# facebookresearch/actionmesh

Measured on NVIDIA H100. Metric: denoiser_steps_per_sec, higher is better.
Workload: dtype bf16

## Files before the change

### actionmesh_b200/csrc/attention.cu

```cuda
#include "common.cuh"
#include "ptx.cuh"
#include "attention.cuh"

namespace amb {

constexpr int ATT_BQ = 128;
constexpr int ATT_BK = 128;
constexpr int ATT_THREADS = 384;
constexpr int ATT_STAGES = 2;

template <int D>
struct AttnSmem {
  static constexpr int BOX_BYTES = 128 * 128;
  static constexpr int Q_BYTES = (D / 64) * BOX_BYTES;
  static constexpr int KV_BYTES = (D / 64) * BOX_BYTES;
  static constexpr int Q_OFF = 0;
  static constexpr int K_OFF = Q_BYTES;
  static constexpr int V_OFF = K_OFF + ATT_STAGES * KV_BYTES;
  static constexpr int BAR_OFF = V_OFF + ATT_STAGES * KV_BYTES;
  static constexpr int NUM_BARS = 1 + 4 * ATT_STAGES;
  static constexpr int TOTAL = BAR_OFF + NUM_BARS * 8 + 1024;
};

template <int D>
__device__ __forceinline__ void qk_issue(float* sc, uint32_t sq_addr, uint32_t sk_addr) {
#pragma unroll
  for (int k = 0; k < D / 16; ++k) {
    const uint32_t off = (k >> 2) * AttnSmem<D>::BOX_BYTES + (k & 3) * 32;
    wgmma_ss_n128(sc, make_desc_kmajor_sw128(sq_addr + off), make_desc_kmajor_sw128(sk_addr + off), k > 0 ? 1u : 0u);
  }
  wgmma_commit();
}

template <int D>
__device__ __forceinline__ void pv_issue(float* o, const uint32_t* pk, uint32_t sv_addr) {
#pragma unroll
  for (int kk = 0; kk < ATT_BK / 16; ++kk) {
    const uint64_t vdesc = make_desc_mnmajor_sw128(sv_addr + kk * 2048, AttnSmem<D>::BOX_BYTES);
    if constexpr (D == 128) wgmma_rs_n128_tb(o, pk + 4 * kk, vdesc, 1u);
    else wgmma_rs_n64_tb(o, pk + 4 * kk, vdesc, 1u);
  }
  wgmma_commit();
}

__device__ __forceinline__ void softmax_tile(float* sc, int valid, int q, float c, float& m_a, float& m_b, float& l_a,
                                             float& l_b, float& al_a, float& al_b) {
  if (valid < ATT_BK) {
#pragma unroll
    for (int i = 0; i < 16; ++i) {
      const int key = 8 * i + 2 * q;
      if (key >= valid) sc[4 * i] = sc[4 * i + 2] = -INFINITY;
      if (key + 1 >= valid) sc[4 * i + 1] = sc[4 * i + 3] = -INFINITY;
    }
  }
  float mx_a = m_a, mx_b = m_b;
#pragma unroll
  for (int i = 0; i < 16; ++i) {
    mx_a = fmaxf(mx_a, fmaxf(sc[4 * i], sc[4 * i + 1]));
    mx_b = fmaxf(mx_b, fmaxf(sc[4 * i + 2], sc[4 * i + 3]));
  }
  mx_a = fmaxf(mx_a, __shfl_xor_sync(0xffffffffu, mx_a, 1));
  mx_b = fmaxf(mx_b, __shfl_xor_sync(0xffffffffu, mx_b, 1));
  mx_a = fmaxf(mx_a, __shfl_xor_sync(0xffffffffu, mx_a, 2));
  mx_b = fmaxf(mx_b, __shfl_xor_sync(0xffffffffu, mx_b, 2));
  al_a = ex2_approx((m_a - mx_a) * c);
  al_b = ex2_approx((m_b - mx_b) * c);
  m_a = mx_a;
  m_b = mx_b;
  const float mb_a = m_a * c, mb_b = m_b * c;
  float ts_a = 0.f, ts_b = 0.f;
#pragma unroll
  for (int i = 0; i < 16; ++i) {
    sc[4 * i] = ex2_approx(fmaf(sc[4 * i], c, -mb_a));
    sc[4 * i + 1] = ex2_approx(fmaf(sc[4 * i + 1], c, -mb_a));
    sc[4 * i + 2] = ex2_approx(fmaf(sc[4 * i + 2], c, -mb_b));
    sc[4 * i + 3] = ex2_approx(fmaf(sc[4 * i + 3], c, -mb_b));
    ts_a += sc[4 * i] + sc[4 * i + 1];
    ts_b += sc[4 * i + 2] + sc[4 * i + 3];
  }
  l_a = l_a * al_a + ts_a;
  l_b = l_b * al_b + ts_b;
}

__device__ __forceinline__ void pack_p(uint32_t* pk, const float* sc) {
#pragma unroll
  for (int i = 0; i < 16; ++i) {
    pk[2 * i] = pack_bf16(sc[4 * i], sc[4 * i + 1]);
    pk[2 * i + 1] = pack_bf16(sc[4 * i + 2], sc[4 * i + 3]);
  }
}

template <int D>
__global__ void __launch_bounds__(ATT_THREADS, 1)
flash_attn_fwd_kernel(const __grid_constant__ CUtensorMap tmQ, const __grid_constant__ CUtensorMap tmK,
                      const __grid_constant__ CUtensorMap tmV, const AttnParams p) {
  using L = AttnSmem<D>;
  constexpr int DH = D / 64;
  extern __shared__ uint8_t smem_raw[];
  uint8_t* smem = reinterpret_cast<uint8_t*>((reinterpret_cast<uintptr_t>(smem_raw) + 1023) & ~uintptr_t(1023));
  uint64_t* q_full = reinterpret_cast<uint64_t*>(smem + L::BAR_OFF);
  uint64_t* k_full = q_full + 1;
  uint64_t* v_full = k_full + ATT_STAGES;
  uint64_t* k_empty = v_full + ATT_STAGES;
  uint64_t* v_empty = k_empty + ATT_STAGES;

  const int wg = __shfl_sync(0xffffffffu, threadIdx.x >> 7, 0);
  const int warp = threadIdx.x >> 5;
  const int lane = threadIdx.x & 31;
  const int q0 = blockIdx.x * ATT_BQ;
  const int head = blockIdx.y;
  const int batch = blockIdx.z;
  const int tiles_per_chunk = (p.sk_chunk + ATT_BK - 1) / ATT_BK;
  const int n_kv = p.kv_chunks * tiles_per_chunk;

  if (threadIdx.x == 0) {
    tma_prefetch_desc(&tmQ);
    tma_prefetch_desc(&tmK);
    tma_prefetch_desc(&tmV);
    mbar_init(q_full, 1);
    for (int s = 0; s < ATT_STAGES; ++s) {
      mbar_init(&k_full[s], 1);
      mbar_init(&v_full[s], 1);
      mbar_init(&k_empty[s], 8);
      mbar_init(&v_empty[s], 8);
    }
    fence_mbar_init();
  }
  __syncthreads();

  if (wg == 0) {
    reg_dealloc<24>();
    if (warp == 0) {
      if (elect_one()) {
        mbar_expect_tx(q_full, L::Q_BYTES);
        for (int c = 0; c < DH; ++c)
          tma_load_4d(smem + L::Q_OFF + c * L::BOX_BYTES, &tmQ, q_full, c * 64, q0, head, batch, kEvictFirst);
      }
      __syncwarp();
      int s = 0;
      uint32_t phase = 0;
      for (int j = 0; j < n_kv; ++j) {
        const int chunk = j / tiles_per_chunk;
        const int key0 = (j - chunk * tiles_per_chunk) * ATT_BK;
        mbar_wait(&k_empty[s], phase ^ 1);
        if (elect_one()) {
          uint8_t* sk = smem + L::K_OFF + s * L::KV_BYTES;
          mbar_expect_tx(&k_full[s], L::KV_BYTES);
          for (int c = 0; c < DH; ++c)
            tma_load_5d(sk + c * L::BOX_BYTES, &tmK, &k_full[s], c * 64, key0, head, batch, chunk, kEvictLast);
        }
        __syncwarp();
        mbar_wait(&v_empty[s], phase ^ 1);
        if (elect_one()) {
          uint8_t* sv = smem + L::V_OFF + s * L::KV_BYTES;
          mbar_expect_tx(&v_full[s], L::KV_BYTES);
          for (int c = 0; c < DH; ++c)
            tma_load_5d(sv + c * L::BOX_BYTES, &tmV, &v_full[s], c * 64, key0, head, batch, chunk, kEvictLast);
        }
        __syncwarp();
        if (++s == ATT_STAGES) { s = 0; phase ^= 1; }
      }
      for (int j = 0; j < ATT_STAGES; ++j) {
        mbar_wait(&k_empty[s], phase ^ 1);
        mbar_wait(&v_empty[s], phase ^ 1);
        if (++s == ATT_STAGES) { s = 0; phase ^= 1; }
      }
    }
  } else {
    reg_alloc<240>();
    const int q = lane & 3;
    const int r_local = (wg - 1) * 64 + (warp & 3) * 16 + (lane >> 2);
    const uint32_t sq_addr = smem_u32(smem + L::Q_OFF) + (wg - 1) * 64 * 128;
    const uint32_t sk_addr = smem_u32(smem + L::K_OFF);
    const uint32_t sv_addr = smem_u32(smem + L::V_OFF);
    const float c = p.scale_log2;
    const int last_valid = p.sk_chunk - (tiles_per_chunk - 1) * ATT_BK;
    const uint32_t my_turn = wg, other_turn = 3 - wg;

    float o[D / 2];
#pragma unroll
    for (int i = 0; i < D / 2; ++i) o[i] = 0.f;
    float m_a = -INFINITY, m_b = -INFINITY;
    float l_a = 0.f, l_b = 0.f;
    float al_a, al_b;
    float sc[64];
    uint32_t pk[32];

    mbar_wait_watched(q_full, 0);
    mbar_wait_watched(&k_full[0], 0);
    if (wg == 2) named_bar_sync(my_turn, 256);
    wgmma_fence();
    qk_issue<D>(sc, sq_addr, sk_addr);
    named_bar_arrive(other_turn, 256);
    wgmma_wait<0>();
#pragma unroll
    for (int i = 0; i < 64; ++i) reg_fence(sc[i]);
    __syncwarp();
    if (lane == 0) mbar_arrive(&k_empty[0]);
    int jn = tiles_per_chunk == 1 ? 0 : 1;
    softmax_tile(sc, tiles_per_chunk == 1 ? last_valid : ATT_BK, q, c, m_a, m_b, l_a, l_b, al_a, al_b);
    pack_p(pk, sc);

    int s = 0;
    uint32_t phase = 0;
    for (int j = 0; j + 1 < n_kv; ++j) {
      int sn = s + 1;
      uint32_t phn = phase;
      if (sn == ATT_STAGES) { sn = 0; phn ^= 1; }
      mbar_wait_watched(&k_full[sn], phn);
      mbar_wait_watched(&v_full[s], phase);
      named_bar_sync(my_turn, 256);
      wgmma_fence();
      qk_issue<D>(sc, sq_addr, sk_addr + sn * L::KV_BYTES);
      pv_issue<D>(o, pk, sv_addr + s * L::KV_BYTES);
      named_bar_arrive(other_turn, 256);
      wgmma_wait<1>();
#pragma unroll
      for (int i = 0; i < 64; ++i) reg_fence(sc[i]);
      __syncwarp();
      if (lane == 0) mbar_arrive(&k_empty[sn]);
      softmax_tile(sc, jn == tiles_per_chunk - 1 ? last_valid : ATT_BK, q, c, m_a, m_b, l_a, l_b, al_a, al_b);
      if (++jn == tiles_per_chunk) jn = 0;
      wgmma_wait<0>();
#pragma unroll
      for (int i = 0; i < D / 2; ++i) reg_fence(o[i]);
      __syncwarp();
      if (lane == 0) mbar_arrive(&v_empty[s]);
#pragma unroll
      for (int i = 0; i < D / 8; ++i) {
        o[4 * i] *= al_a;
        o[4 * i + 1] *= al_a;
        o[4 * i + 2] *= al_b;
        o[4 * i + 3] *= al_b;
      }
      pack_p(pk, sc);
      s = sn;
      phase = phn;
    }

    mbar_wait_watched(&v_full[s], phase);
    named_bar_sync(my_turn, 256);
    wgmma_fence();
    pv_issue<D>(o, pk, sv_addr + s * L::KV_BYTES);
    if (wg == 1) named_bar_arrive(other_turn, 256);
    wgmma_wait<0>();
#pragma unroll
    for (int i = 0; i < D / 2; ++i) reg_fence(o[i]);
    __syncwarp();
    if (lane == 0) mbar_arrive(&v_empty[s]);

    l_a += __shfl_xor_sync(0xffffffffu, l_a, 1);
    l_b += __shfl_xor_sync(0xffffffffu, l_b, 1);
    l_a += __shfl_xor_sync(0xffffffffu, l_a, 2);
    l_b += __shfl_xor_sync(0xffffffffu, l_b, 2);
    const float inv_a = 1.0f / l_a, inv_b = 1.0f / l_b;
    const int qr_a = q0 + r_local, qr_b = qr_a + 8;
    __nv_bfloat16* obase = p.o + (long long)batch * p.o_stride_b + (long long)head * p.o_stride_h + 2 * q;
#pragma unroll
    for (int i = 0; i < D / 8; ++i) {
      if (qr_a < p.sq)
        *reinterpret_cast<uint32_t*>(obase + (long long)qr_a * p.o_stride_s + 8 * i) = pack_bf16(o[4 * i] * inv_a, o[4 * i + 1] * inv_a);
      if (qr_b < p.sq)
        *reinterpret_cast<uint32_t*>(obase + (long long)qr_b * p.o_stride_s + 8 * i) = pack_bf16(o[4 * i + 2] * inv_b, o[4 * i + 3] * inv_b);
    }
  }
}

template <int D>
static int launch_attn(const amb_attn_args* a, cudaStream_t stream) {
  using L = AttnSmem<D>;
  CUtensorMap tmQ, tmK, tmV;
  int r = encode_attn_maps(a, D, ATT_BQ, ATT_BK, ATT_BK, &tmQ, &tmK, &tmV);
  if (r) return r;
  const AttnParams p = make_attn_params(a);
  dim3 grid((a->sq + ATT_BQ - 1) / ATT_BQ, a->heads, a->batch);
  auto kern = flash_attn_fwd_kernel<D>;
  r = ensure_smem_optin(kern, L::TOTAL);
  if (r) return r;
  kern<<<grid, ATT_THREADS, L::TOTAL, stream>>>(tmQ, tmK, tmV, p);
  AMB_CHECK_CUDA(cudaGetLastError());
  return AMB_OK;
}

}

using namespace amb;

extern "C" int amb_flash_attn_fwd(const amb_attn_args* a, amb_stream_t stream) {
  AMB_CHECK_ARG(a && a->q && a->k && a->v && a->o, "flash_attn: null pointer");
  AMB_CHECK_ARG(a->batch > 0 && a->heads > 0 && a->sq > 0 && a->sk > 0, "flash_attn: bad shape b=%d h=%d sq=%d sk=%d",
                a->batch, a->heads, a->sq, a->sk);
  AMB_CHECK_ARG(a->head_dim == 128 || a->head_dim == 64, "flash_attn: head_dim %d unsupported (64 or 128)", a->head_dim);
  AMB_CHECK_ARG(a->q_stride_s % 8 == 0 && a->k_stride_s % 8 == 0 && a->v_stride_s % 8 == 0 && a->o_stride_s % 8 == 0 &&
                    a->q_stride_h % 8 == 0 && a->k_stride_h % 8 == 0 && a->v_stride_h % 8 == 0 && a->o_stride_h % 8 == 0 &&
                    a->q_stride_b % 8 == 0 && a->k_stride_b % 8 == 0 && a->v_stride_b % 8 == 0 && a->o_stride_b % 8 == 0,
                "flash_attn: strides must be multiples of 8 elements (16 bytes)");
  AMB_CHECK_ARG(a->kv_chunks <= 1 || (a->sk_chunk > 0 && (int64_t)a->sk_chunk * a->kv_chunks == a->sk),
                "flash_attn: kv_chunks * sk_chunk must equal sk");
  AMB_CHECK_ARG(a->batch <= 65535 && a->heads <= 65535, "flash_attn: grid limits");
  cudaStream_t s = (cudaStream_t)stream;
  if (a->head_dim == 64) return launch_attn<64>(a, s);
  return launch_attn<128>(a, s);
}
```

### actionmesh_b200/csrc/ptx.cuh

```cuda
#pragma once
#include <cstdint>
#include <cuda_runtime.h>
#include <cuda_bf16.h>

namespace amb {

__device__ __forceinline__ uint32_t smem_u32(const void* p) {
  return static_cast<uint32_t>(__cvta_generic_to_shared(p));
}
__device__ __forceinline__ uint32_t lane_id() { return threadIdx.x & 31; }

__device__ __forceinline__ bool elect_one() {
  uint32_t pred = 0;
  asm volatile(
      "{\n\t.reg .pred P;\n\t"
      "elect.sync _|P, 0xffffffff;\n\t"
      "selp.u32 %0, 1, 0, P;\n\t}\n"
      : "=r"(pred));
  return pred != 0;
}

__device__ __forceinline__ void mbar_init(uint64_t* bar, uint32_t count) {
  asm volatile("mbarrier.init.shared::cta.b64 [%0], %1;" ::"r"(smem_u32(bar)), "r"(count) : "memory");
}
__device__ __forceinline__ void fence_mbar_init() {
  asm volatile("fence.mbarrier_init.release.cluster;" ::: "memory");
}
__device__ __forceinline__ void fence_proxy_async_smem() {
  asm volatile("fence.proxy.async.shared::cta;" ::: "memory");
}
__device__ __forceinline__ void mbar_expect_tx(uint64_t* bar, uint32_t bytes) {
  asm volatile("mbarrier.arrive.expect_tx.shared::cta.b64 _, [%0], %1;" ::"r"(smem_u32(bar)), "r"(bytes)
               : "memory");
}
__device__ __forceinline__ void mbar_arrive(uint64_t* bar) {
  asm volatile("mbarrier.arrive.shared::cta.b64 _, [%0];" ::"r"(smem_u32(bar)) : "memory");
}
__device__ __forceinline__ uint32_t mbar_try_wait(uint64_t* bar, uint32_t parity) {
  uint32_t ok;
  asm volatile(
      "{\n\t.reg .pred P;\n\t"
      "mbarrier.try_wait.parity.shared::cta.b64 P, [%1], %2;\n\t"
      "selp.u32 %0, 1, 0, P;\n\t}\n"
      : "=r"(ok)
      : "r"(smem_u32(bar)), "r"(parity)
      : "memory");
  return ok;
}
__device__ __forceinline__ void mbar_arrive_cluster(uint64_t* bar, uint32_t cta) {
  asm volatile(
      "{\n\t.reg .b32 ra;\n\t"
      "mapa.shared::cluster.u32 ra, %0, %1;\n\t"
      "mbarrier.arrive.shared::cluster.b64 _, [ra];\n\t}\n"
      ::"r"(smem_u32(bar)), "r"(cta)
      : "memory");
}

__device__ __forceinline__ uint32_t cluster_ctarank() {
  uint32_t r;
  asm volatile("mov.u32 %0, %%cluster_ctarank;" : "=r"(r));
  return r;
}
__device__ __forceinline__ void cluster_sync() {
  asm volatile("barrier.cluster.arrive.release;\n\tbarrier.cluster.wait.acquire;" ::: "memory");
}
__device__ __forceinline__ uint64_t globaltimer_ns() {
  uint64_t t;
  asm volatile("mov.u64 %0, %%globaltimer;" : "=l"(t));
  return t;
}
#ifndef AMB_WAIT_TIMEOUT_NS
#define AMB_WAIT_TIMEOUT_NS 4000000000ull
#endif
#ifndef AMB_WAIT_TIMEOUT_PRINT
#define AMB_WAIT_TIMEOUT_PRINT 0
#endif
__device__ __forceinline__ void mbar_wait(uint64_t* bar, uint32_t parity) {
  if (mbar_try_wait(bar, parity)) return;
  uint64_t t0 = globaltimer_ns();
  uint32_t spins = 0;
  while (!mbar_try_wait(bar, parity)) {
    if ((++spins & 0xfff) == 0 && globaltimer_ns() - t0 > AMB_WAIT_TIMEOUT_NS) {
#if AMB_WAIT_TIMEOUT_PRINT
      printf("amb: mbarrier wait timeout block=(%d,%d,%d) thread=%d bar=%u parity=%u\n", blockIdx.x, blockIdx.y,
             blockIdx.z, threadIdx.x, smem_u32(bar), parity);
#endif
      __trap();
    }
  }
}
__device__ __forceinline__ void mbar_wait_watched(uint64_t* bar, uint32_t parity) {
  while (!mbar_try_wait(bar, parity)) {
  }
}

__device__ __forceinline__ void tma_prefetch_desc(const void* tmap) {
  asm volatile("prefetch.tensormap [%0];" ::"l"(reinterpret_cast<uint64_t>(tmap)) : "memory");
}
constexpr uint64_t kEvictNormal = 0x1000000000000000ull;
constexpr uint64_t kEvictFirst = 0x12F0000000000000ull;
constexpr uint64_t kEvictLast = 0x14F0000000000000ull;

__device__ __forceinline__ void tma_load_2d(void* dst, const void* tmap, uint64_t* bar, int c0, int c1,
                                            uint64_t hint) {
  asm volatile(
      "cp.async.bulk.tensor.2d.shared::cluster.global.mbarrier::complete_tx::bytes.L2::cache_hint"
      " [%0], [%1, {%3, %4}], [%2], %5;"
      :
      : "r"(smem_u32(dst)), "l"(reinterpret_cast<uint64_t>(tmap)), "r"(smem_u32(bar)), "r"(c0), "r"(c1), "l"(hint)
      : "memory");
}
__device__ __forceinline__ void tma_load_2d_multicast(void* dst, const void* tmap, uint64_t* bar, int c0, int c1,
                                                      uint16_t cta_mask, uint64_t hint) {
  asm volatile(
      "cp.async.bulk.tensor.2d.shared::cluster.global.mbarrier::complete_tx::bytes.multicast::cluster.L2::cache_hint"
      " [%0], [%1, {%4, %5}], [%2], %3, %6;"
      :
      : "r"(smem_u32(dst)), "l"(reinterpret_cast<uint64_t>(tmap)), "r"(smem_u32(bar)), "h"(cta_mask), "r"(c0), "r"(c1),
        "l"(hint)
      : "memory");
}
__device__ __forceinline__ void tma_load_4d(void* dst, const void* tmap, uint64_t* bar, int c0, int c1, int c2,
                                            int c3, uint64_t hint) {
  asm volatile(
      "cp.async.bulk.tensor.4d.shared::cluster.global.mbarrier::complete_tx::bytes.L2::cache_hint"
      " [%0], [%1, {%3, %4, %5, %6}], [%2], %7;"
      :
      : "r"(smem_u32(dst)), "l"(reinterpret_cast<uint64_t>(tmap)), "r"(smem_u32(bar)), "r"(c0), "r"(c1), "r"(c2),
        "r"(c3), "l"(hint)
      : "memory");
}

__device__ __forceinline__ void tma_load_5d(void* dst, const void* tmap, uint64_t* bar, int c0, int c1, int c2,
                                            int c3, int c4, uint64_t hint) {
  asm volatile(
      "cp.async.bulk.tensor.5d.shared::cluster.global.mbarrier::complete_tx::bytes.L2::cache_hint"
      " [%0], [%1, {%3, %4, %5, %6, %7}], [%2], %8;"
      :
      : "r"(smem_u32(dst)), "l"(reinterpret_cast<uint64_t>(tmap)), "r"(smem_u32(bar)), "r"(c0), "r"(c1), "r"(c2),
        "r"(c3), "r"(c4), "l"(hint)
      : "memory");
}

__device__ __forceinline__ void wgmma_fence() { asm volatile("wgmma.fence.sync.aligned;" ::: "memory"); }
__device__ __forceinline__ void wgmma_commit() { asm volatile("wgmma.commit_group.sync.aligned;" ::: "memory"); }
template <int N>
__device__ __forceinline__ void wgmma_wait() {
  asm volatile("wgmma.wait_group.sync.aligned %0;" ::"n"(N) : "memory");
}
__device__ __forceinline__ void reg_fence(float& r) { asm volatile("" : "+f"(r)::"memory"); }

__device__ __forceinline__ uint64_t make_smem_desc(uint32_t saddr, uint32_t lbo_bytes, uint32_t sbo_bytes) {
  uint64_t d = 0;
  d |= static_cast<uint64_t>((saddr & 0x3FFFF) >> 4);
  d |= static_cast<uint64_t>((lbo_bytes >> 4) & 0x3FFF) << 16;
  d |= static_cast<uint64_t>((sbo_bytes >> 4) & 0x3FFF) << 32;
  d |= 1ull << 62;
  return d;
}
__device__ __forceinline__ uint64_t make_desc_kmajor_sw128(uint32_t saddr) { return make_smem_desc(saddr, 16, 1024); }
__device__ __forceinline__ uint64_t make_desc_mnmajor_sw128(uint32_t saddr, uint32_t lbo_bytes) {
  return make_smem_desc(saddr, lbo_bytes, 1024);
}

__device__ __forceinline__ void wgmma_ss_n64(float* d, uint64_t desc_a, uint64_t desc_b, uint32_t scale_d) {
  asm volatile(
      "{\n\t.reg .pred p;\n\tsetp.ne.b32 p, %34, 0;\n\t"
      "wgmma.mma_async.sync.aligned.m64n64k16.f32.bf16.bf16 {%0, %1, %2, %3, %4, %5, %6, %7, %8, %9, %10, %11, %12, %13, %14, %15, %16, %17, %18, %19, %20, %21, %22, %23, %24, %25, %26, %27, %28, %29, %30, %31}, %32, %33, p, 1, 1, 0, 0;\n\t}\n"
      : "+f"(d[0]), "+f"(d[1]), "+f"(d[2]), "+f"(d[3]), "+f"(d[4]), "+f"(d[5]), "+f"(d[6]), "+f"(d[7]), "+f"(d[8]), "+f"(d[9]), "+f"(d[10]), "+f"(d[11]), "+f"(d[12]), "+f"(d[13]), "+f"(d[14]), "+f"(d[15]), "+f"(d[16]), "+f"(d[17]), "+f"(d[18]), "+f"(d[19]), "+f"(d[20]), "+f"(d[21]), "+f"(d[22]), "+f"(d[23]), "+f"(d[24]), "+f"(d[25]), "+f"(d[26]), "+f"(d[27]), "+f"(d[28]), "+f"(d[29]), "+f"(d[30]), "+f"(d[31])
      : "l"(desc_a), "l"(desc_b), "r"(scale_d));
}
__device__ __forceinline__ void wgmma_ss_n128(float* d, uint64_t desc_a, uint64_t desc_b, uint32_t scale_d) {
  asm volatile(
      "{\n\t.reg .pred p;\n\tsetp.ne.b32 p, %66, 0;\n\t"
      "wgmma.mma_async.sync.aligned.m64n128k16.f32.bf16.bf16 {%0, %1, %2, %3, %4, %5, %6, %7, %8, %9, %10, %11, %12, %13, %14, %15, %16, %17, %18, %19, %20, %21, %22, %23, %24, %25, %26, %27, %28, %29, %30, %31, %32, %33, %34, %35, %36, %37, %38, %39, %40, %41, %42, %43, %44, %45, %46, %47, %48, %49, %50, %51, %52, %53, %54, %55, %56, %57, %58, %59, %60, %61, %62, %63}, %64, %65, p, 1, 1, 0, 0;\n\t}\n"
      : "+f"(d[0]), "+f"(d[1]), "+f"(d[2]), "+f"(d[3]), "+f"(d[4]), "+f"(d[5]), "+f"(d[6]), "+f"(d[7]), "+f"(d[8]), "+f"(d[9]), "+f"(d[10]), "+f"(d[11]), "+f"(d[12]), "+f"(d[13]), "+f"(d[14]), "+f"(d[15]), "+f"(d[16]), "+f"(d[17]), "+f"(d[18]), "+f"(d[19]), "+f"(d[20]), "+f"(d[21]), "+f"(d[22]), "+f"(d[23]), "+f"(d[24]), "+f"(d[25]), "+f"(d[26]), "+f"(d[27]), "+f"(d[28]), "+f"(d[29]), "+f"(d[30]), "+f"(d[31]), "+f"(d[32]), "+f"(d[33]), "+f"(d[34]), "+f"(d[35]), "+f"(d[36]), "+f"(d[37]), "+f"(d[38]), "+f"(d[39]), "+f"(d[40]), "+f"(d[41]), "+f"(d[42]), "+f"(d[43]), "+f"(d[44]), "+f"(d[45]), "+f"(d[46]), "+f"(d[47]), "+f"(d[48]), "+f"(d[49]), "+f"(d[50]), "+f"(d[51]), "+f"(d[52]), "+f"(d[53]), "+f"(d[54]), "+f"(d[55]), "+f"(d[56]), "+f"(d[57]), "+f"(d[58]), "+f"(d[59]), "+f"(d[60]), "+f"(d[61]), "+f"(d[62]), "+f"(d[63])
      : "l"(desc_a), "l"(desc_b), "r"(scale_d));
}
__device__ __forceinline__ void wgmma_ss_n256(float* d, uint64_t desc_a, uint64_t desc_b, uint32_t scale_d) {
  asm volatile(
      "{\n\t.reg .pred p;\n\tsetp.ne.b32 p, %130, 0;\n\t"
      "wgmma.mma_async.sync.aligned.m64n256k16.f32.bf16.bf16 {%0, %1, %2, %3, %4, %5, %6, %7, %8, %9, %10, %11, %12, %13, %14, %15, %16, %17, %18, %19, %20, %21, %22, %23, %24, %25, %26, %27, %28, %29, %30, %31, %32, %33, %34, %35, %36, %37, %38, %39, %40, %41, %42, %43, %44, %45, %46, %47, %48, %49, %50, %51, %52, %53, %54, %55, %56, %57, %58, %59, %60, %61, %62, %63, %64, %65, %66, %67, %68, %69, %70, %71, %72, %73, %74, %75, %76, %77, %78, %79, %80, %81, %82, %83, %84, %85, %86, %87, %88, %89, %90, %91, %92, %93, %94, %95, %96, %97, %98, %99, %100, %101, %102, %103, %104, %105, %106, %107, %108, %109, %110, %111, %112, %113, %114, %115, %116, %117, %118, %119, %120, %121, %122, %123, %124, %125, %126, %127}, %128, %129, p, 1, 1, 0, 0;\n\t}\n"
      : "+f"(d[0]), "+f"(d[1]), "+f"(d[2]), "+f"(d[3]), "+f"(d[4]), "+f"(d[5]), "+f"(d[6]), "+f"(d[7]), "+f"(d[8]), "+f"(d[9]), "+f"(d[10]), "+f"(d[11]), "+f"(d[12]), "+f"(d[13]), "+f"(d[14]), "+f"(d[15]), "+f"(d[16]), "+f"(d[17]), "+f"(d[18]), "+f"(d[19]), "+f"(d[20]), "+f"(d[21]), "+f"(d[22]), "+f"(d[23]), "+f"(d[24]), "+f"(d[25]), "+f"(d[26]), "+f"(d[27]), "+f"(d[28]), "+f"(d[29]), "+f"(d[30]), "+f"(d[31]), "+f"(d[32]), "+f"(d[33]), "+f"(d[34]), "+f"(d[35]), "+f"(d[36]), "+f"(d[37]), "+f"(d[38]), "+f"(d[39]), "+f"(d[40]), "+f"(d[41]), "+f"(d[42]), "+f"(d[43]), "+f"(d[44]), "+f"(d[45]), "+f"(d[46]), "+f"(d[47]), "+f"(d[48]), "+f"(d[49]), "+f"(d[50]), "+f"(d[51]), "+f"(d[52]), "+f"(d[53]), "+f"(d[54]), "+f"(d[55]), "+f"(d[56]), "+f"(d[57]), "+f"(d[58]), "+f"(d[59]), "+f"(d[60]), "+f"(d[61]), "+f"(d[62]), "+f"(d[63]), "+f"(d[64]), "+f"(d[65]), "+f"(d[66]), "+f"(d[67]), "+f"(d[68]), "+f"(d[69]), "+f"(d[70]), "+f"(d[71]), "+f"(d[72]), "+f"(d[73]), "+f"(d[74]), "+f"(d[75]), "+f"(d[76]), "+f"(d[77]), "+f"(d[78]), "+f"(d[79]), "+f"(d[80]), "+f"(d[81]), "+f"(d[82]), "+f"(d[83]), "+f"(d[84]), "+f"(d[85]), "+f"(d[86]), "+f"(d[87]), "+f"(d[88]), "+f"(d[89]), "+f"(d[90]), "+f"(d[91]), "+f"(d[92]), "+f"(d[93]), "+f"(d[94]), "+f"(d[95]), "+f"(d[96]), "+f"(d[97]), "+f"(d[98]), "+f"(d[99]), "+f"(d[100]), "+f"(d[101]), "+f"(d[102]), "+f"(d[103]), "+f"(d[104]), "+f"(d[105]), "+f"(d[106]), "+f"(d[107]), "+f"(d[108]), "+f"(d[109]), "+f"(d[110]), "+f"(d[111]), "+f"(d[112]), "+f"(d[113]), "+f"(d[114]), "+f"(d[115]), "+f"(d[116]), "+f"(d[117]), "+f"(d[118]), "+f"(d[119]), "+f"(d[120]), "+f"(d[121]), "+f"(d[122]), "+f"(d[123]), "+f"(d[124]), "+f"(d[125]), "+f"(d[126]), "+f"(d[127])
      : "l"(desc_a), "l"(desc_b), "r"(scale_d));
}
__device__ __forceinline__ void wgmma_rs_n64_tb(float* d, const uint32_t* a, uint64_t desc_b, uint32_t scale_d) {
  asm volatile(
      "{\n\t.reg .pred p;\n\tsetp.ne.b32 p, %37, 0;\n\t"
      "wgmma.mma_async.sync.aligned.m64n64k16.f32.bf16.bf16 {%0, %1, %2, %3, %4, %5, %6, %7, %8, %9, %10, %11, %12, %13, %14, %15, %16, %17, %18, %19, %20, %21, %22, %23, %24, %25, %26, %27, %28, %29, %30, %31}, {%32, %33, %34, %35}, %36, p, 1, 1, 1;\n\t}\n"
      : "+f"(d[0]), "+f"(d[1]), "+f"(d[2]), "+f"(d[3]), "+f"(d[4]), "+f"(d[5]), "+f"(d[6]), "+f"(d[7]), "+f"(d[8]), "+f"(d[9]), "+f"(d[10]), "+f"(d[11]), "+f"(d[12]), "+f"(d[13]), "+f"(d[14]), "+f"(d[15]), "+f"(d[16]), "+f"(d[17]), "+f"(d[18]), "+f"(d[19]), "+f"(d[20]), "+f"(d[21]), "+f"(d[22]), "+f"(d[23]), "+f"(d[24]), "+f"(d[25]), "+f"(d[26]), "+f"(d[27]), "+f"(d[28]), "+f"(d[29]), "+f"(d[30]), "+f"(d[31])
      : "r"(a[0]), "r"(a[1]), "r"(a[2]), "r"(a[3]), "l"(desc_b), "r"(scale_d));
}
__device__ __forceinline__ void wgmma_rs_n128_tb(float* d, const uint32_t* a, uint64_t desc_b, uint32_t scale_d) {
  asm volatile(
      "{\n\t.reg .pred p;\n\tsetp.ne.b32 p, %69, 0;\n\t"
      "wgmma.mma_async.sync.aligned.m64n128k16.f32.bf16.bf16 {%0, %1, %2, %3, %4, %5, %6, %7, %8, %9, %10, %11, %12, %13, %14, %15, %16, %17, %18, %19, %20, %21, %22, %23, %24, %25, %26, %27, %28, %29, %30, %31, %32, %33, %34, %35, %36, %37, %38, %39, %40, %41, %42, %43, %44, %45, %46, %47, %48, %49, %50, %51, %52, %53, %54, %55, %56, %57, %58, %59, %60, %61, %62, %63}, {%64, %65, %66, %67}, %68, p, 1, 1, 1;\n\t}\n"
      : "+f"(d[0]), "+f"(d[1]), "+f"(d[2]), "+f"(d[3]), "+f"(d[4]), "+f"(d[5]), "+f"(d[6]), "+f"(d[7]), "+f"(d[8]), "+f"(d[9]), "+f"(d[10]), "+f"(d[11]), "+f"(d[12]), "+f"(d[13]), "+f"(d[14]), "+f"(d[15]), "+f"(d[16]), "+f"(d[17]), "+f"(d[18]), "+f"(d[19]), "+f"(d[20]), "+f"(d[21]), "+f"(d[22]), "+f"(d[23]), "+f"(d[24]), "+f"(d[25]), "+f"(d[26]), "+f"(d[27]), "+f"(d[28]), "+f"(d[29]), "+f"(d[30]), "+f"(d[31]), "+f"(d[32]), "+f"(d[33]), "+f"(d[34]), "+f"(d[35]), "+f"(d[36]), "+f"(d[37]), "+f"(d[38]), "+f"(d[39]), "+f"(d[40]), "+f"(d[41]), "+f"(d[42]), "+f"(d[43]), "+f"(d[44]), "+f"(d[45]), "+f"(d[46]), "+f"(d[47]), "+f"(d[48]), "+f"(d[49]), "+f"(d[50]), "+f"(d[51]), "+f"(d[52]), "+f"(d[53]), "+f"(d[54]), "+f"(d[55]), "+f"(d[56]), "+f"(d[57]), "+f"(d[58]), "+f"(d[59]), "+f"(d[60]), "+f"(d[61]), "+f"(d[62]), "+f"(d[63])
      : "r"(a[0]), "r"(a[1]), "r"(a[2]), "r"(a[3]), "l"(desc_b), "r"(scale_d));
}

__device__ __forceinline__ void named_bar_sync(uint32_t id, uint32_t nthreads) {
  asm volatile("bar.sync %0, %1;" ::"r"(id), "r"(nthreads) : "memory");
}
__device__ __forceinline__ void named_bar_arrive(uint32_t id, uint32_t nthreads) {
  asm volatile("bar.arrive %0, %1;" ::"r"(id), "r"(nthreads) : "memory");
}

template <int N>
__device__ __forceinline__ void reg_alloc() {
  asm volatile("setmaxnreg.inc.sync.aligned.u32 %0;" ::"n"(N));
}
template <int N>
__device__ __forceinline__ void reg_dealloc() {
  asm volatile("setmaxnreg.dec.sync.aligned.u32 %0;" ::"n"(N));
}
__device__ __forceinline__ float ex2_approx(float x) {
  float y;
  asm("ex2.approx.ftz.f32 %0, %1;" : "=f"(y) : "f"(x));
  return y;
}
__device__ __forceinline__ uint32_t pack_bf16(float lo, float hi) {
  __nv_bfloat162 v = __floats2bfloat162_rn(lo, hi);
  return *reinterpret_cast<uint32_t*>(&v);
}
__device__ __forceinline__ float2 unpack_bf16(uint32_t u) {
  __nv_bfloat162 v = *reinterpret_cast<__nv_bfloat162*>(&u);
  return __bfloat1622float2(v);
}

}
```

Before: 1.092.

## Multicast K/V tiles across 2-CTA clusters in flash attention for long KV

Adds a clustered variant of the attention kernel in which two CTAs that share a head split the K/V tile loads and multicast each half to both CTAs, with the empty-slot barriers counting arrivals from both CTAs. It is used only when there are at least 64 KV tiles, and is meant to halve the L2-to-SM traffic per CTA for K and V. In exchange it adds cluster synchronisation and cross-CTA barrier coupling. A padded CTA whose query tile is out of range must still consume and release slots, and cluster scheduling constraints may reduce occupancy flexibility.

```diff
diff --git a/actionmesh_b200/csrc/attention.cu b/actionmesh_b200/csrc/attention.cu
--- a/actionmesh_b200/csrc/attention.cu
+++ b/actionmesh_b200/csrc/attention.cu
@@ -8,6 +8,8 @@
 constexpr int ATT_BK = 128;
 constexpr int ATT_THREADS = 384;
 constexpr int ATT_STAGES = 2;
+constexpr int ATT_CLUSTER = 2;
+constexpr int ATT_PAIR_MIN_KV_TILES = 64;
 
 template <int D>
 struct AttnSmem {
@@ -90,7 +92,16 @@
   }
 }
 
-template <int D>
+template <bool PAIR>
+__device__ __forceinline__ void release_slot(uint64_t* bar, int lane) {
+  if constexpr (PAIR) {
+    if (lane < ATT_CLUSTER) mbar_arrive_cluster(bar, lane);
+  } else {
+    if (lane == 0) mbar_arrive(bar);
+  }
+}
+
+template <int D, bool PAIR>
 __global__ void __launch_bounds__(ATT_THREADS, 1)
 flash_attn_fwd_kernel(const __grid_constant__ CUtensorMap tmQ, const __grid_constant__ CUtensorMap tmK,
                       const __grid_constant__ CUtensorMap tmV, const AttnParams p) {
@@ -107,6 +118,8 @@
   const int wg = __shfl_sync(0xffffffffu, threadIdx.x >> 7, 0);
   const int warp = threadIdx.x >> 5;
   const int lane = threadIdx.x & 31;
+  constexpr int NCTA = PAIR ? ATT_CLUSTER : 1;
+  const uint32_t rank = PAIR ? cluster_ctarank() : 0;
   const int q0 = blockIdx.x * ATT_BQ;
   const int head = blockIdx.y;
   const int batch = blockIdx.z;
@@ -121,17 +134,18 @@
     for (int s = 0; s < ATT_STAGES; ++s) {
       mbar_init(&k_full[s], 1);
       mbar_init(&v_full[s], 1);
-      mbar_init(&k_empty[s], 8);
-      mbar_init(&v_empty[s], 8);
+      mbar_init(&k_empty[s], 8 * NCTA);
+      mbar_init(&v_empty[s], 8 * NCTA);
     }
     fence_mbar_init();
   }
-  __syncthreads();
+  if constexpr (PAIR) cluster_sync();
+  else __syncthreads();
 
   if (wg == 0) {
     reg_dealloc<24>();
     if (warp == 0) {
-      if (elect_one()) {
+      if ((!PAIR || q0 < p.sq) && elect_one()) {
         mbar_expect_tx(q_full, L::Q_BYTES);
         for (int c = 0; c < DH; ++c)
           tma_load_4d(smem + L::Q_OFF + c * L::BOX_BYTES, &tmQ, q_full, c * 64, q0, head, batch, kEvictFirst);
@@ -139,6 +153,9 @@
       __syncwarp();
       int s = 0;
       uint32_t phase = 0;
+      constexpr uint16_t kPair = (1u << ATT_CLUSTER) - 1;
+      const bool load_k = DH == 2 || rank == 0, load_v = DH == 2 || rank == 1;
+      const int cr = DH == 2 ? (int)rank : 0;
       for (int j = 0; j < n_kv; ++j) {
         const int chunk = j / tiles_per_chunk;
         const int key0 = (j - chunk * tiles_per_chunk) * ATT_BK;
@@ -146,16 +163,28 @@
         if (elect_one()) {
           uint8_t* sk = smem + L::K_OFF + s * L::KV_BYTES;
           mbar_expect_tx(&k_full[s], L::KV_BYTES);
-          for (int c = 0; c < DH; ++c)
-            tma_load_5d(sk + c * L::BOX_BYTES, &tmK, &k_full[s], c * 64, key0, head, batch, chunk, kEvictLast);
+          if constexpr (PAIR) {
+            if (load_k)
+              tma_load_5d_multicast(sk + cr * L::BOX_BYTES, &tmK, &k_full[s], cr * 64, key0, head, batch, chunk, kPair,
+                                    kEvictLast);
+          } else {
+            for (int c = 0; c < DH; ++c)
+              tma_load_5d(sk + c * L::BOX_BYTES, &tmK, &k_full[s], c * 64, key0, head, batch, chunk, kEvictLast);
+          }
         }
         __syncwarp();
         mbar_wait(&v_empty[s], phase ^ 1);
         if (elect_one()) {
           uint8_t* sv = smem + L::V_OFF + s * L::KV_BYTES;
           mbar_expect_tx(&v_full[s], L::KV_BYTES);
-          for (int c = 0; c < DH; ++c)
-            tma_load_5d(sv + c * L::BOX_BYTES, &tmV, &v_full[s], c * 64, key0, head, batch, chunk, kEvictLast);
+          if constexpr (PAIR) {
+            if (load_v)
+              tma_load_5d_multicast(sv + cr * L::BOX_BYTES, &tmV, &v_full[s], cr * 64, key0, head, batch, chunk, kPair,
+                                    kEvictLast);
+          } else {
+            for (int c = 0; c < DH; ++c)
+              tma_load_5d(sv + c * L::BOX_BYTES, &tmV, &v_full[s], c * 64, key0, head, batch, chunk, kEvictLast);
+          }
         }
         __syncwarp();
         if (++s == ATT_STAGES) { s = 0; phase ^= 1; }
@@ -165,6 +194,18 @@
         mbar_wait(&v_empty[s], phase ^ 1);
         if (++s == ATT_STAGES) { s = 0; phase ^= 1; }
       }
+    }
+  } else if (PAIR && q0 >= p.sq) {
+    int s = 0;
+    uint32_t phase = 0;
+    for (int j = 0; j < n_kv; ++j) {
+      mbar_wait_watched(&k_full[s], phase);
+      __syncwarp();
+      release_slot<PAIR>(&k_empty[s], lane);
+      mbar_wait_watched(&v_full[s], phase);
+      __syncwarp();
+      release_slot<PAIR>(&v_empty[s], lane);
+      if (++s == ATT_STAGES) { s = 0; phase ^= 1; }
     }
   } else {
     reg_alloc<240>();
@@ -196,7 +237,7 @@
 #pragma unroll
     for (int i = 0; i < 64; ++i) reg_fence(sc[i]);
     __syncwarp();
-    if (lane == 0) mbar_arrive(&k_empty[0]);
+    release_slot<PAIR>(&k_empty[0], lane);
     int jn = tiles_per_chunk == 1 ? 0 : 1;
     softmax_tile(sc, tiles_per_chunk == 1 ? last_valid : ATT_BK, q, c, m_a, m_b, l_a, l_b, al_a, al_b);
     pack_p(pk, sc);
@@ -218,14 +259,14 @@
 #pragma unroll
       for (int i = 0; i < 64; ++i) reg_fence(sc[i]);
       __syncwarp();
-      if (lane == 0) mbar_arrive(&k_empty[sn]);
+      release_slot<PAIR>(&k_empty[sn], lane);
       softmax_tile(sc, jn == tiles_per_chunk - 1 ? last_valid : ATT_BK, q, c, m_a, m_b, l_a, l_b, al_a, al_b);
       if (++jn == tiles_per_chunk) jn = 0;
       wgmma_wait<0>();
 #pragma unroll
       for (int i = 0; i < D / 2; ++i) reg_fence(o[i]);
       __syncwarp();
-      if (lane == 0) mbar_arrive(&v_empty[s]);
+      release_slot<PAIR>(&v_empty[s], lane);
 #pragma unroll
       for (int i = 0; i < D / 8; ++i) {
         o[4 * i] *= al_a;
@@ -247,7 +288,7 @@
 #pragma unroll
     for (int i = 0; i < D / 2; ++i) reg_fence(o[i]);
     __syncwarp();
-    if (lane == 0) mbar_arrive(&v_empty[s]);
+    release_slot<PAIR>(&v_empty[s], lane);
 
     l_a += __shfl_xor_sync(0xffffffffu, l_a, 1);
     l_b += __shfl_xor_sync(0xffffffffu, l_b, 1);
@@ -264,22 +305,51 @@
         *reinterpret_cast<uint32_t*>(obase + (long long)qr_b * p.o_stride_s + 8 * i) = pack_bf16(o[4 * i + 2] * inv_b, o[4 * i + 3] * inv_b);
     }
   }
+  if constexpr (PAIR) {
+    __syncwarp();
+    cluster_sync();
+  }
+}
+
+template <int D, bool PAIR>
+static int launch_kernel(const CUtensorMap& tmQ, const CUtensorMap& tmK, const CUtensorMap& tmV, const AttnParams& p,
+                         int q_tiles, int heads, int batch, cudaStream_t stream) {
+  using L = AttnSmem<D>;
+  auto kern = flash_attn_fwd_kernel<D, PAIR>;
+  int r = ensure_smem_optin(kern, L::TOTAL);
+  if (r) return r;
+  if constexpr (PAIR) {
+    cudaLaunchConfig_t cfg = {};
+    cfg.gridDim = dim3((q_tiles + ATT_CLUSTER - 1) / ATT_CLUSTER * ATT_CLUSTER, heads, batch);
+    cfg.blockDim = dim3(ATT_THREADS, 1, 1);
+    cfg.dynamicSmemBytes = L::TOTAL;
+    cfg.stream = stream;
+    cudaLaunchAttribute attr[1];
+    attr[0].id = cudaLaunchAttributeClusterDimension;
+    attr[0].val.clusterDim.x = ATT_CLUSTER;
+    attr[0].val.clusterDim.y = 1;
+    attr[0].val.clusterDim.z = 1;
+    cfg.attrs = attr;
+    cfg.numAttrs = 1;
+    AMB_CHECK_CUDA(cudaLaunchKernelEx(&cfg, kern, tmQ, tmK, tmV, p));
+  } else {
+    kern<<<dim3(q_tiles, heads, batch), ATT_THREADS, L::TOTAL, stream>>>(tmQ, tmK, tmV, p);
+    AMB_CHECK_CUDA(cudaGetLastError());
+  }
+  return AMB_OK;
 }
 
 template <int D>
 static int launch_attn(const amb_attn_args* a, cudaStream_t stream) {
-  using L = AttnSmem<D>;
   CUtensorMap tmQ, tmK, tmV;
   int r = encode_attn_maps(a, D, ATT_BQ, ATT_BK, ATT_BK, &tmQ, &tmK, &tmV);
   if (r) return r;
   const AttnParams p = make_attn_params(a);
-  dim3 grid((a->sq + ATT_BQ - 1) / ATT_BQ, a->heads, a->batch);
-  auto kern = flash_attn_fwd_kernel<D>;
-  r = ensure_smem_optin(kern, L::TOTAL);
-  if (r) return r;
-  kern<<<grid, ATT_THREADS, L::TOTAL, stream>>>(tmQ, tmK, tmV, p);
-  AMB_CHECK_CUDA(cudaGetLastError());
-  return AMB_OK;
+  const int q_tiles = (a->sq + ATT_BQ - 1) / ATT_BQ;
+  const int kv_tiles = p.kv_chunks * ((p.sk_chunk + ATT_BK - 1) / ATT_BK);
+  if (kv_tiles >= ATT_PAIR_MIN_KV_TILES)
+    return launch_kernel<D, true>(tmQ, tmK, tmV, p, q_tiles, a->heads, a->batch, stream);
+  return launch_kernel<D, false>(tmQ, tmK, tmV, p, q_tiles, a->heads, a->batch, stream);
 }
 
 }
diff --git a/actionmesh_b200/csrc/ptx.cuh b/actionmesh_b200/csrc/ptx.cuh
--- a/actionmesh_b200/csrc/ptx.cuh
+++ b/actionmesh_b200/csrc/ptx.cuh
@@ -141,6 +141,16 @@
         "r"(c3), "r"(c4), "l"(hint)
       : "memory");
 }
+__device__ __forceinline__ void tma_load_5d_multicast(void* dst, const void* tmap, uint64_t* bar, int c0, int c1, int c2,
+                                                      int c3, int c4, uint16_t cta_mask, uint64_t hint) {
+  asm volatile(
+      "cp.async.bulk.tensor.5d.shared::cluster.global.mbarrier::complete_tx::bytes.multicast::cluster.L2::cache_hint"
+      " [%0], [%1, {%4, %5, %6, %7, %8}], [%2], %3, %9;"
+      :
+      : "r"(smem_u32(dst)), "l"(reinterpret_cast<uint64_t>(tmap)), "r"(smem_u32(bar)), "h"(cta_mask), "r"(c0), "r"(c1),
+        "r"(c2), "r"(c3), "r"(c4), "l"(hint)
+      : "memory");
+}
 
 __device__ __forceinline__ void wgmma_fence() { asm volatile("wgmma.fence.sync.aligned;" ::: "memory"); }
 __device__ __forceinline__ void wgmma_commit() { asm volatile("wgmma.commit_group.sync.aligned;" ::: "memory"); }
```

Measured after the change: 1.113 (median of 6 runs). 1.02x the previous value.
